# TritonDataCenter/containerpilot

Hardware: AMD Instinct MI355X
Metric: events/sec (higher is better)
Workload: dtype n/a (CPU daemon, no tensor math; see BASELINE.json north_star); 1 GPU; model=containerpilot daemon, BASELINE stress shape scaled to 550 jobs, jobs=550, watches=50, parallelism=1 independent daemons (1/rank)

## Files before the change

cpp/include/cpilot/discovery.hpp:

```cpp
#pragma once

#include <condition_variable>
#include <deque>
#include <functional>
#include <map>
#include <memory>
#include <set>
#include <mutex>
#include <string>
#include <thread>
#include <vector>

#include "cpilot/http.hpp"
#include "cpilot/json.hpp"
#include "cpilot/kv.hpp"
#include "cpilot/loop.hpp"
#include "cpilot/metrics.hpp"

namespace cpilot {

struct ServiceEntry {
  std::string id;
  std::string address;
  int port = 0;
  std::vector<std::string> tags;
  std::string node;
  std::string nodeAddress;
};

std::vector<ServiceEntry> parseHealthEntries(const std::string& body,
                                             bool* ok);

std::string kvRequestPath(const std::string& key, bool prefix,
                          const std::string& dc, bool blocking = false,
                          uint64_t index = 0, int waitSeconds = 0);

class ConsulBackend {
 public:
  static std::unique_ptr<ConsulBackend> create(const Json* raw,
                                               std::string* err);

  ~ConsulBackend();

  void start(Loop& loop);
  void stop();

  using DoneCb = std::function<void(bool ok, const std::string& err)>;
  using HealthCb =
      std::function<void(bool ok, std::vector<ServiceEntry> entries)>;
  using HealthBlockingCb = std::function<void(
      bool ok, std::vector<ServiceEntry> entries, uint64_t index)>;

  void serviceRegister(const std::string& id, const std::string& name,
                       const std::vector<std::string>& tags, int port,
                       const std::string& address, bool enableTagOverride,
                       int ttlSeconds, const std::string& status,
                       const std::string& deregisterAfter, DoneCb cb);
  void updateTTL(const std::string& checkID, const std::string& output,
                 const std::string& status, DoneCb cb);
  void serviceDeregister(const std::string& id, DoneCb cb);
  void healthService(const std::string& name, const std::string& tag,
                     const std::string& dc, HealthCb cb);

  void healthServiceBlocking(const std::string& name, const std::string& tag,
                             const std::string& dc, uint64_t lastIndex,
                             int waitSeconds, HealthBlockingCb cb);

  bool compareAndSwap(const std::string& service,
                      std::vector<ServiceEntry> entries);

  using KVCb = std::function<void(bool ok, std::vector<KVEntry> entries)>;
  using KVBlockingCb = std::function<void(
      bool ok, std::vector<KVEntry> entries, uint64_t index)>;
  void kvGet(const std::string& key, bool prefix, const std::string& dc,
             KVCb cb);
  void kvGetBlocking(const std::string& key, bool prefix,
                     const std::string& dc, uint64_t lastIndex,
                     int waitSeconds, KVBlockingCb cb);
  bool compareAndSwapKV(const std::string& watch,
                        std::vector<KVEntry> entries);

  const std::string& address() const { return address_; }
  const std::string& scheme() const { return scheme_; }

  std::shared_ptr<prom::Family> watchGauge() { return watchGauge_; }

 private:
  ConsulBackend() = default;
  void workerMain();
  bool enqueue(const std::string& key, std::function<void()> task);
  using BlockingFinish = std::function<std::function<void()>(
      const http::ClientResult& res, bool live, uint64_t index)>;
  bool startBlockingGet(const std::string& path, int waitSeconds,
                        size_t maxBody, BlockingFinish finish);

  std::string address_;
  std::string scheme_ = "http";
  std::string token_;
  http::TlsOptions tls_;

  Loop* loop_ = nullptr;
  std::vector<std::thread> workers_;
  std::deque<std::pair<std::string, std::function<void()>>> tasks_;
  std::set<std::string> queuedKeys_;
  uint64_t dropped_ = 0;
  std::mutex mu_;
  std::condition_variable cv_;
  bool stopping_ = false;

  std::map<std::string, std::vector<ServiceEntry>> watched_;
  std::map<std::string, std::vector<KVEntry>> watchedKV_;
  std::shared_ptr<prom::Family> watchGauge_;

  struct BlockingReg {
    std::mutex mu;
    std::set<std::shared_ptr<http::CancelToken>> tokens;
    bool stopping = false;
  };
  std::shared_ptr<BlockingReg> blockingReg_ =
      std::make_shared<BlockingReg>();
};

struct ServiceDefinition
    : public std::enable_shared_from_this<ServiceDefinition> {
  std::string id;
  std::string name;
  int port = 0;
  int ttl = 0;
  std::vector<std::string> tags;
  std::string initialStatus;
  std::string ipAddress;
  bool enableTagOverride = false;
  std::string deregisterCriticalServiceAfter;
  ConsulBackend* consul = nullptr;

  bool wasRegistered = false;
  bool registerInFlight = false;

  void sendHeartbeat();
  void registerWithInitialStatus();
  void deregister();
  void markForMaintenance();

 private:
  void registerService(const std::string& status);
};

}
```

cpp/include/cpilot/http.hpp:

```cpp
#pragma once

#include <sys/socket.h>

#include <functional>
#include <map>
#include <mutex>
#include <memory>
#include <string>

#include "cpilot/loop.hpp"

namespace cpilot {
namespace http {

struct Request {
  std::string method;
  std::string path;
  std::string query;
  std::map<std::string, std::string> headers;
  std::string body;
};

struct Response {
  int status = 200;
// ... 61 lines not shown
class CancelToken {
 public:
  void arm(int fd);
  void disarm();
  void cancel();
  bool cancelled();

 private:
  std::mutex mu_;
  int fd_ = -1;
  bool cancelled_ = false;
};

struct TlsOptions {
  bool enabled = false;
  std::string caFile;
  std::string caPath;
  std::string certFile;
  std::string keyFile;
  std::string serverName;
  bool insecureSkipVerify = false;
};

extern const char* const kBodyTooLarge;

ClientResult request(const std::string& target, const std::string& method,
                     const std::string& path, const std::string& body,
                     const std::string& contentType = "application/json",
                     const std::map<std::string, std::string>& headers = {},
                     int timeoutMs = 10000,
                     const TlsOptions* tls = nullptr,
                     CancelToken* cancel = nullptr, size_t maxBody = 0);

}
}
```

cpp/include/cpilot/loop.hpp:

```cpp
#pragma once

#include <sys/types.h>

#include <chrono>
#include <cstdint>
#include <deque>
#include <functional>
#include <map>
#include <memory>
#include <mutex>
#include <queue>
#include <vector>

namespace cpilot {

using Clock = std::chrono::steady_clock;
using TimePoint = Clock::time_point;
using Ns = std::chrono::nanoseconds;

std::function<void()> timedItem(const char* tag, std::function<void()> fn);
void dumpItemTags();

void resetThreadScheduling();

class Loop {
 public:
  using FdCallback = std::function<void(uint32_t epollEvents)>;
  using TimerCallback = std::function<void()>;
  using ChildCallback = std::function<void(int waitStatus)>;

  Loop();
  ~Loop();

  Loop(const Loop&) = delete;
  Loop& operator=(const Loop&) = delete;

  void watchFd(int fd, uint32_t events, FdCallback cb);
  void modifyFd(int fd, uint32_t events);
  void unwatchFd(int fd);

  uint64_t addTimeout(Ns delay, TimerCallback cb);
  uint64_t addInterval(Ns interval, TimerCallback cb, Ns initialDelay = Ns(-1));
  void cancelTimer(uint64_t id);

  void defer(std::function<void()> fn);

  void post(std::function<void()> fn);

  void watchChild(pid_t pid, ChildCallback cb);
  void reapChildren();
  void notifyChildExit(pid_t pid, int status);

  static void postIfLive(Loop* loop, uint64_t id, std::function<void()> fn);
  uint64_t id() const { return id_; }

  void run();
  void stop();

  bool stopped() const { return stopped_; }

 private:
  struct Timer {
    uint64_t id;
    TimePoint deadline;
    Ns interval;
    TimerCallback cb;
    bool canceled = false;
  };
  struct TimerCmp {
    bool operator()(const std::shared_ptr<Timer>& a,
                    const std::shared_ptr<Timer>& b) const {
      return a->deadline > b->deadline;
    }
  };

  void armTimerFd();
  void fireDueTimers();
  void drainDeferred();
  void drainPosted();

  uint64_t id_ = 0;
  int epfd_ = -1;
  int timerfd_ = -1;
  int wakeupFds_[2] = {-1, -1};
  bool stopped_ = false;

  std::map<int, FdCallback> fdCallbacks_;
  std::priority_queue<std::shared_ptr<Timer>,
                      std::vector<std::shared_ptr<Timer>>, TimerCmp>
      timers_;
  std::map<uint64_t, std::shared_ptr<Timer>> timersById_;
  uint64_t nextTimerId_ = 1;

  std::deque<std::function<void()>> deferred_;

  std::mutex postedMu_;
  std::deque<std::function<void()>> posted_;

  std::map<pid_t, ChildCallback> children_;
  std::map<pid_t, int> unclaimedExits_;
};

}
```

cpp/include/cpilot/spawner.hpp:

```cpp
#pragma once

#include <sys/types.h>

#include <cstdint>
#include <deque>
#include <functional>
#include <map>
#include <memory>
#include <mutex>
#include <string>
#include <thread>
#include <vector>

#include "cpilot/loop.hpp"

namespace cpilot {

class Spawner {
 public:
  using SpawnCb = std::function<void(pid_t pid, int err)>;

  static Spawner& global();

  void spawn(Loop& loop, const std::string& execPath,
             const std::vector<std::string>& args,
             std::shared_ptr<const std::vector<std::string>> baseEnv,
             const std::vector<std::string>& extraEnv, int stdioFd,
             SpawnCb cb);

  int helperCount() const { return (int)helpers_.size(); }

  size_t backlog();
  bool overloaded();

 private:
  Spawner();
  struct Helper {
    int sock = -1;
    pid_t pid = -1;
    bool dead = false;
    std::deque<std::pair<std::vector<char>, int>> overflow;
    std::mutex sendMu;
  };
  struct Pending {
    Loop* loop;
    uint64_t loopId;
    SpawnCb cb;
    size_t helperIdx;
  };

  bool launchHelper(Helper* h);
  void flushOverflow(size_t idx);
  void readerMain();
  void handleMessage(size_t idx, const char* buf, size_t len);
  void helperDied(size_t idx);
  bool sendRequest(Helper& h, const std::vector<char>& buf, int fd);
  void wakeReader();

  std::string helperPath_;
  std::vector<std::unique_ptr<Helper>> helpers_;
  size_t nextHelper_ = 0;

  std::mutex mu_;
  std::map<uint32_t, Pending> pending_;
  uint32_t nextReqId_ = 1;
  std::map<pid_t, std::pair<Loop*, uint64_t>> pidLoops_;

  int wakeFds_[2] = {-1, -1};
  std::thread reader_;
};

}
```

cpp/src/discovery.cpp:

```cpp
#include "cpilot/discovery.hpp"

#include <algorithm>
#include <cstdlib>
#include <thread>

#include "cpilot/decode.hpp"
#include "cpilot/http.hpp"
#include "cpilot/log.hpp"

namespace cpilot {

namespace {

void parseRawURI(const std::string& raw, std::string* address,
                 std::string* scheme) {
  *scheme = "http";
  *address = raw;
  if (raw.rfind("http://", 0) == 0) {
    *address = raw.substr(7);
  } else if (raw.rfind("https://", 0) == 0) {
    *address = raw.substr(8);
    *scheme = "https";
  }
}

std::string urlEncode(const std::string& s) {
  std::string out;
  for (unsigned char c : s) {
    if (isalnum(c) || c == '-' || c == '_' || c == '.' || c == '~' ||
        c == ':' || c == '@') {
      out += c;
    } else {
      char buf[4];
// ... 93 lines not shown
  if (const char* v = getenv("CONSUL_CACERT"))
    if (v[0]) backend->tls_.caFile = v;
  if (const char* v = getenv("CONSUL_CAPATH"))
    if (v[0]) backend->tls_.caPath = v;
  if (const char* v = getenv("CONSUL_CLIENT_CERT"))
    if (v[0]) backend->tls_.certFile = v;
  if (const char* v = getenv("CONSUL_CLIENT_KEY"))
    if (v[0]) backend->tls_.keyFile = v;
  if (const char* v = getenv("CONSUL_TLS_SERVER_NAME"))
    if (v[0]) backend->tls_.serverName = v;
  if (const char* v = getenv("CONSUL_HTTP_SSL_VERIFY")) {
    std::string s2(v);
    for (auto& ch : s2) ch = tolower(ch);
    if (s2 == "1" || s2 == "true") backend->tls_.insecureSkipVerify = false;
    else if (s2 == "0" || s2 == "false")
      backend->tls_.insecureSkipVerify = true;
  }
  backend->tls_.enabled = (backend->scheme_ == "https");
  backend->watchGauge_ = prom::Registry::global().registerFamily(
      "containerpilot_watch_instances",
      "gauge of instances found for each ContainerPilot watch, partitioned "
      "by service",
      prom::MetricType::Gauge, {"service"});
  return backend;
}

ConsulBackend::~ConsulBackend() { stop(); }

void ConsulBackend::start(Loop& loop) {
  loop_ = &loop;
  stopping_ = false;
  if (blockingReg_->stopping)
    blockingReg_ = std::make_shared<BlockingReg>();
  for (int i = 0; i < 4; i++)
    workers_.emplace_back([this] { workerMain(); });
}

void ConsulBackend::stop() {
  {
    std::lock_guard<std::mutex> l(mu_);
    if (stopping_ && workers_.empty()) return;
    stopping_ = true;
  }
  {
    std::lock_guard<std::mutex> l(blockingReg_->mu);
    blockingReg_->stopping = true;
    for (auto& t : blockingReg_->tokens) t->cancel();
  }
  cv_.notify_all();
  for (auto& t : workers_) t.join();
  workers_.clear();
}

void ConsulBackend::workerMain() {
  resetThreadScheduling();
  while (true) {
    std::function<void()> task;
    {
      std::unique_lock<std::mutex> l(mu_);
      cv_.wait(l, [this] { return stopping_ || !tasks_.empty(); });
      if (stopping_ && tasks_.empty()) return;
      auto& front = tasks_.front();
      if (!front.first.empty()) queuedKeys_.erase(front.first);
      task = std::move(front.second);
      tasks_.pop_front();
    }
    task();
  }
}

bool ConsulBackend::enqueue(const std::string& key,
                            std::function<void()> task) {
  {
    std::lock_guard<std::mutex> l(mu_);
    if (stopping_) return false;
    if (!key.empty() && !queuedKeys_.insert(key).second) return false;
    if (tasks_.size() >= 10000) {
      if (++dropped_ % 1000 == 1)
        LOG_WARN("consul task queue full, dropping requests (%llu dropped)",
                 (unsigned long long)dropped_);
      if (!key.empty()) queuedKeys_.erase(key);
      return false;
    }
    tasks_.emplace_back(key, std::move(task));
  }
  cv_.notify_one();
  return true;
}
// ... 15 lines not shown
  payload.emplace_back("ID", Json(id));
  payload.emplace_back("Name", Json(name));
  if (!tags.empty()) {
    JsonArray tagArr;
    for (auto& t : tags) tagArr.push_back(Json(t));
    payload.emplace_back("Tags", Json(std::move(tagArr)));
  }
  payload.emplace_back("Port", Json((int64_t)port));
  payload.emplace_back("Address", Json(address));
  if (enableTagOverride)
    payload.emplace_back("EnableTagOverride", Json(true));
  payload.emplace_back("Check", Json(std::move(check)));
  std::string body = Json(std::move(payload)).dump();

  std::string target = address_;
  std::string token = token_;
  http::TlsOptions tls = tls_;
  Loop* loop = loop_;
  bool accepted = enqueue("reg:" + id, [target, token, tls, body, cb, loop] {
    std::map<std::string, std::string> headers;
    if (!token.empty()) headers["X-Consul-Token"] = token;
    auto res = http::request(target, "PUT", "/v1/agent/service/register",
                             body, "application/json", headers, 10000, &tls);
    bool ok = res.ok && res.status == 200;
    std::string err = res.ok ? ("status " + std::to_string(res.status) + ": " +
                                res.body)
                             : res.error;
    loop->post(timedItem("consul", [cb, ok, err] { cb(ok, ok ? "" : err); }));
  });
  if (!accepted)
    loop_->post([cb] { cb(false, "request coalesced or queue full"); });
}

void ConsulBackend::updateTTL(const std::string& checkID,
                              const std::string& output,
                              const std::string& status, DoneCb cb) {
  std::string st = status;
  if (st == "pass") st = "passing";
  else if (st == "warn") st = "warning";
  else if (st == "fail") st = "critical";
  JsonObject payload;
  payload.emplace_back("Status", Json(st));
  payload.emplace_back("Output", Json(output));
  std::string body = Json(std::move(payload)).dump();
  std::string path = "/v1/agent/check/update/" + urlEncode(checkID);

  std::string target = address_;
  std::string token = token_;
  http::TlsOptions tls = tls_;
  Loop* loop = loop_;
  bool accepted =
      enqueue("ttl:" + checkID, [target, token, tls, path, body, cb, loop] {
    std::map<std::string, std::string> headers;
    if (!token.empty()) headers["X-Consul-Token"] = token;
    auto res = http::request(target, "PUT", path, body, "application/json",
                             headers, 10000, &tls);
    bool ok = res.ok && res.status == 200;
    std::string err =
        res.ok ? ("status " + std::to_string(res.status) + ": " + res.body)
               : res.error;
    loop->post(timedItem("consul", [cb, ok, err] { cb(ok, ok ? "" : err); }));
  });
  if (!accepted) {
    (void)cb;
  }
}

void ConsulBackend::serviceDeregister(const std::string& id, DoneCb cb) {
  std::string path = "/v1/agent/service/deregister/" + urlEncode(id);
  std::string target = address_;
  std::string token = token_;
  http::TlsOptions tls = tls_;
  Loop* loop = loop_;
  bool accepted = enqueue("", [target, token, tls, path, cb, loop] {
    std::map<std::string, std::string> headers;
    if (!token.empty()) headers["X-Consul-Token"] = token;
    auto res = http::request(target, "PUT", path, "", "application/json",
                             headers, 10000, &tls);
    bool ok = res.ok && res.status == 200;
    std::string err =
        res.ok ? ("status " + std::to_string(res.status)) : res.error;
    loop->post(timedItem("consul", [cb, ok, err] { cb(ok, ok ? "" : err); }));
  });
  if (!accepted) loop_->post([cb] { cb(false, "queue full"); });
}

std::vector<ServiceEntry> parseHealthEntries(const std::string& body,
                                             bool* ok) {
  std::vector<ServiceEntry> entries;
  try {
    Json doc = parseJson5(body);
    if (doc.isArray()) {
      for (auto& e : doc.array()) {
        const Json* svc = e.find("Service");
        if (!svc || !svc->isObject()) continue;
        ServiceEntry entry;
        if (const Json* v = svc->find("ID"))
          if (v->isString()) entry.id = v->str();
// ... 185 lines not shown
      });
  if (!started) loop_->post([cb] { cb(false, {}, 0); });
}

bool ConsulBackend::compareAndSwapKV(const std::string& watch,
                                     std::vector<KVEntry> entries) {
  std::vector<KVEntry>& cached = watchedKV_[watch];
  bool changed = kvEntriesDiffer(cached, entries);
  cached = std::move(entries);
  return changed;
}

bool ConsulBackend::compareAndSwap(const std::string& service,
                                   std::vector<ServiceEntry> entries) {
  std::vector<ServiceEntry> existing = watched_[service];
  watched_[service] = entries;
  if (existing.size() != entries.size()) return true;
  auto byID = [](const ServiceEntry& a, const ServiceEntry& b) {
    return a.id < b.id;
  };
  std::sort(existing.begin(), existing.end(), byID);
  std::sort(entries.begin(), entries.end(), byID);
  for (size_t i = 0; i < existing.size(); i++) {
    if (existing[i].address != entries[i].address ||
        existing[i].port != entries[i].port)
      return true;
  }
  return false;
}


void ServiceDefinition::sendHeartbeat() {
  registerService("passing");
  std::string checkID = "service:" + id;
  consul->updateTTL(checkID, "ok", "pass", [](bool ok, const std::string& err) {
    if (!ok) LOG_WARN("service update TTL failed: %s", err.c_str());
  });
}

void ServiceDefinition::registerWithInitialStatus() {
  if (wasRegistered) return;
  std::string status;
  if (initialStatus == "passing") status = "passing";
  else if (initialStatus == "warning") status = "warning";
  else if (initialStatus == "critical") status = "critical";
  LOG_INFO("Registering service %s with initial status set to %s",
           name.c_str(), initialStatus.c_str());
  registerService(status);
}

void ServiceDefinition::registerService(const std::string& status) {
  if (wasRegistered || registerInFlight) return;
  registerInFlight = true;
  std::weak_ptr<ServiceDefinition> weak = weak_from_this();
  consul->serviceRegister(
      id, name, tags, port, ipAddress, enableTagOverride, ttl, status,
      deregisterCriticalServiceAfter,
      [weak](bool ok, const std::string& err) {
        auto self = weak.lock();
        if (!self) return;
        self->registerInFlight = false;
        if (!ok) {
          LOG_WARN("service registration failed: %s", err.c_str());
          return;
        }
        LOG_INFO("Service registered: %s", self->name.c_str());
        self->wasRegistered = true;
      });
}

// ... 11 lines not shown
```

cpp/src/http.cpp:

```cpp
#include "cpilot/http.hpp"

#include <sys/epoll.h>

#include <arpa/inet.h>
#include <fcntl.h>
#include <netdb.h>
#include <netinet/in.h>
#include <netinet/tcp.h>
#include <poll.h>
#include <openssl/err.h>
#include <openssl/ssl.h>
#include <sys/socket.h>
#include <sys/un.h>
#include <unistd.h>

#include <cctype>
#include <cstring>

#include "cpilot/log.hpp"

namespace cpilot {
namespace http {

const char* statusText(int code) {
// ... 432 lines not shown
         SSL_CTX_use_PrivateKey_file(ctx, tls.keyFile.c_str(),
                                     SSL_FILETYPE_PEM) != 1)) {
      *err = "failed to load client certificate/key";
      return false;
    }
    SSL_CTX_set_verify(
        ctx, tls.insecureSkipVerify ? SSL_VERIFY_NONE : SSL_VERIFY_PEER,
        nullptr);
    ssl = SSL_new(ctx);
    SSL_set_fd(ssl, fd);
    std::string sniHost = tls.serverName.empty() ? host : tls.serverName;
    size_t colon = sniHost.rfind(':');
    if (colon != std::string::npos) sniHost = sniHost.substr(0, colon);
    SSL_set_tlsext_host_name(ssl, sniHost.c_str());
    if (!tls.insecureSkipVerify) SSL_set1_host(ssl, sniHost.c_str());
    if (SSL_connect(ssl) != 1) {
      unsigned long e = ERR_get_error();
      char ebuf[256];
      ERR_error_string_n(e, ebuf, sizeof(ebuf));
      *err = std::string("TLS handshake failed: ") + ebuf;
      return false;
    }
    return true;
  }

  ssize_t send(const char* data, size_t len) {
    return ssl ? SSL_write(ssl, data, (int)len) : write(fd, data, len);
  }
  ssize_t recv(char* data, size_t len) {
    return ssl ? SSL_read(ssl, data, (int)len) : read(fd, data, len);
  }
};

struct ConnPool {
  std::map<std::string, int> conns;
  ~ConnPool() {
    for (auto& kv : conns) close(kv.second);
  }
};
thread_local ConnPool connPool;

int poolTake(const std::string& target) {
  auto it = connPool.conns.find(target);
  if (it == connPool.conns.end()) return -1;
  int fd = it->second;
  connPool.conns.erase(it);
  return fd;
}

void poolStore(const std::string& target, int fd) {
  int& slot = connPool.conns.emplace(target, -1).first->second;
  if (slot >= 0) close(slot);
  slot = fd;
}

bool tryDechunk(const std::string& data, std::string* out) {
  out->clear();
  size_t pos = 0;
  while (true) {
    size_t eol = data.find("\r\n", pos);
    if (eol == std::string::npos) return false;
    long len = strtol(data.substr(pos, eol - pos).c_str(), nullptr, 16);
    if (len < 0) return false;
    if (len == 0) return true;
    if (data.size() < eol + 2 + (size_t)len + 2) return false;
    out->append(data, eol + 2, (size_t)len);
    pos = eol + 2 + (size_t)len + 2;
  }
}

int acquireConn(const std::string& target, int timeoutMs, bool usePool,
                bool* fromPool, std::string* err) {
  int fd = usePool ? poolTake(target) : -1;
  *fromPool = fd >= 0;
  if (fd < 0) fd = connectTarget(target, err);
  if (fd >= 0) setIoTimeout(fd, timeoutMs);
  return fd;
}

std::string serialiseRequest(const std::string& method, const std::string& path,
                             const std::string& host, bool keepAlive,
                             const Headers& headers, const std::string& body,
                             const std::string& contentType) {
  std::string req = method + " " + path + " HTTP/1.1\r\n";
  req += "Host: " + host + "\r\n";
  req += keepAlive ? "Connection: keep-alive\r\n" : "Connection: close\r\n";
  for (auto& kv : headers) req += kv.first + ": " + kv.second + "\r\n";
  if (!body.empty() || method == "POST" || method == "PUT") {
    req += "Content-Type: " + contentType + "\r\n";
    req += "Content-Length: " + std::to_string(body.size()) + "\r\n";
  }
  req += "\r\n";
  req += body;
  return req;
}

bool writeAll(Transport& t, const std::string& data) {
  size_t off = 0;
  while (off < data.size()) {
    ssize_t n = t.send(data.data() + off, data.size() - off);
    if (n > 0)
      off += n;
    else if (!(n < 0 && errno == EINTR && !t.ssl))
      return false;
  }
  return true;
}

bool readMore(Transport& t, std::string* resp) {
  char buf[8192];
// ... 28 lines not shown
  if (isChunked(result->headers)) {
    std::string decoded;
    while (!tryDechunk(resp.substr(bodyStart), &decoded)) {
      if (maxBody && decoded.size() > maxBody) return ReadResult::TooLarge;
      if (!readMore(t, &resp)) return ReadResult::Truncated;
    }
    if (maxBody && decoded.size() > maxBody) return ReadResult::TooLarge;
    result->body = std::move(decoded);
  } else if (result->headers.count("content-length")) {
    size_t want = contentLength(result->headers);
    if (maxBody && want > maxBody) return ReadResult::TooLarge;
    while (resp.size() < bodyStart + want) {
      if (!readMore(t, &resp)) return ReadResult::Truncated;
    }
    result->body = resp.substr(bodyStart, want);
  } else {
    while (readMore(t, &resp)) {
      if (maxBody && resp.size() - bodyStart > maxBody)
        return ReadResult::TooLarge;
    }
    result->body = resp.substr(bodyStart);
    *bodyFramed = false;
  }
  return ReadResult::Ok;
}

bool serverKeepsAlive(const ClientResult& result) {
  auto it = result.headers.find("connection");
  bool closes = it != result.headers.end() &&
                toLower(it->second).find("close") != std::string::npos;
  return !closes && result.status > 0;
}

}

ClientResult request(const std::string& target, const std::string& method,
                     const std::string& path, const std::string& body,
                     const std::string& contentType,
                     const std::map<std::string, std::string>& headers,
                     int timeoutMs, const TlsOptions* tls,
                     CancelToken* cancel, size_t maxBody) {
  ClientResult result;
  if (cancel && cancel->cancelled()) {
    result.error = "cancelled";
    return result;
  }
  const bool tlsOn = tls && tls->enabled;
  const bool reusable = !tlsOn && cancel == nullptr;
  const std::string host =
      target.rfind("unix:", 0) == 0 ? "localhost" : target;
  const std::string req = serialiseRequest(method, path, host, reusable,
                                           headers, body, contentType);

  for (int attempt = 0; attempt < 2; attempt++) {
    result = ClientResult{};
    Transport t;
    bool fromPool = false;
    t.fd = acquireConn(target, timeoutMs, reusable && attempt == 0, &fromPool,
                       &result.error);
    if (t.fd < 0) return result;
    struct Disarm {
      CancelToken* ct;
      ~Disarm() {
        if (ct) ct->disarm();
      }
    } disarm{cancel};
    if (cancel) cancel->arm(t.fd);
    if (tlsOn && !t.startTls(host, *tls, &result.error)) return result;

    if (!writeAll(t, req)) {
      if (fromPool) continue;
      break;
    }
    bool bodyFramed = false;
    ReadResult rr = readResponse(t, &result, &bodyFramed, maxBody);
    if (rr == ReadResult::Empty && fromPool)
      continue;
    if (rr == ReadResult::Empty || rr == ReadResult::Malformed) {
      result.error = (cancel && cancel->cancelled()) ? "cancelled"
                                                     : "malformed response";
      return result;
    }
    if (rr == ReadResult::Truncated) {
      result.error = "truncated response body";
      return result;
    }
    if (rr == ReadResult::TooLarge) {
      result.error = kBodyTooLarge;
      return result;
    }
    result.ok = true;
    if (reusable && bodyFramed && serverKeepsAlive(result)) {
      poolStore(target, t.fd);
      t.fd = -1;
    }
    return result;
  }
  result.error = "write failed";
  return result;
}

}
}
```

cpp/src/loop.cpp:

```cpp
#include "cpilot/loop.hpp"

#include <fcntl.h>
#include <sched.h>
#include <sys/resource.h>
#include <sys/epoll.h>
#include <sys/timerfd.h>
#include <sys/wait.h>
#include <unistd.h>

#include <cstdio>
#include <cstring>
#include <algorithm>
#include <set>
#include <stdexcept>

#include "cpilot/log.hpp"

namespace cpilot {

void resetThreadScheduling() {
  struct sched_param sp;
  memset(&sp, 0, sizeof(sp));
  sched_setscheduler(0, SCHED_OTHER, &sp);
  setpriority(PRIO_PROCESS, 0, 0);
}

namespace {
std::mutex& liveLoopsMu() {
  static std::mutex mu;
  return mu;
}
std::map<Loop*, uint64_t>& liveLoops() {
  static std::map<Loop*, uint64_t> loops;
  return loops;
}
uint64_t nextLoopId() {
  static uint64_t next = 1;
  return next++;
// ... 10 lines not shown
  return tags;
}
}

std::function<void()> timedItem(const char* tag, std::function<void()> fn) {
  static const bool on = cpilotDebugEnv("CPILOT_LOOP_DEBUG");
  if (!on) return fn;
  std::string t(tag);
  return [t, fn = std::move(fn)] {
    TimePoint t0 = Clock::now();
    fn();
    auto& slot = itemTags()[t];
    slot.ms +=
        std::chrono::duration<double, std::milli>(Clock::now() - t0).count();
    slot.count++;
  };
}

void dumpItemTags() {
  for (auto& kv : itemTags())
    fprintf(stderr, "  item tag %s: %.0fms over %llu (avg %.1fus)\n",
            kv.first.c_str(), kv.second.ms,
            (unsigned long long)kv.second.count,
            kv.second.count ? kv.second.ms * 1000 / kv.second.count : 0.0);
  itemTags().clear();
}

void Loop::postIfLive(Loop* loop, uint64_t id, std::function<void()> fn) {
  std::lock_guard<std::mutex> l(liveLoopsMu());
  auto it = liveLoops().find(loop);
  if (it != liveLoops().end() && it->second == id) loop->post(std::move(fn));
}

Loop::Loop() {
  {
    std::lock_guard<std::mutex> l(liveLoopsMu());
    id_ = nextLoopId();
    liveLoops()[this] = id_;
  }
  epfd_ = epoll_create1(EPOLL_CLOEXEC);
  if (epfd_ < 0) throw std::runtime_error("epoll_create1 failed");
  timerfd_ = timerfd_create(CLOCK_MONOTONIC, TFD_NONBLOCK | TFD_CLOEXEC);
  if (timerfd_ < 0) throw std::runtime_error("timerfd_create failed");
  if (pipe2(wakeupFds_, O_NONBLOCK | O_CLOEXEC) != 0)
    throw std::runtime_error("pipe2 failed");

  watchFd(timerfd_, EPOLLIN, [this](uint32_t) {
    uint64_t expirations;
    while (read(timerfd_, &expirations, sizeof(expirations)) > 0) {
    }
    fireDueTimers();
  });
  watchFd(wakeupFds_[0], EPOLLIN, [this](uint32_t) {
    char buf[256];
    while (read(wakeupFds_[0], buf, sizeof(buf)) > 0) {
    }
    drainPosted();
  });
}

Loop::~Loop() {
  {
    std::lock_guard<std::mutex> l(liveLoopsMu());
    liveLoops().erase(this);
  }
  if (epfd_ >= 0) close(epfd_);
  if (timerfd_ >= 0) close(timerfd_);
  if (wakeupFds_[0] >= 0) close(wakeupFds_[0]);
  if (wakeupFds_[1] >= 0) close(wakeupFds_[1]);
}

void Loop::watchFd(int fd, uint32_t events, FdCallback cb) {
  struct epoll_event ev;
  memset(&ev, 0, sizeof(ev));
  ev.events = events;
  ev.data.fd = fd;
  if (epoll_ctl(epfd_, EPOLL_CTL_ADD, fd, &ev) != 0)
    throw std::runtime_error(std::string("epoll_ctl ADD failed: ") +
                             strerror(errno));
  fdCallbacks_[fd] = std::move(cb);
}

void Loop::modifyFd(int fd, uint32_t events) {
  struct epoll_event ev;
  memset(&ev, 0, sizeof(ev));
  ev.events = events;
  ev.data.fd = fd;
  epoll_ctl(epfd_, EPOLL_CTL_MOD, fd, &ev);
}

void Loop::unwatchFd(int fd) {
  epoll_ctl(epfd_, EPOLL_CTL_DEL, fd, nullptr);
  fdCallbacks_.erase(fd);
}

uint64_t Loop::addTimeout(Ns delay, TimerCallback cb) {
  auto t = std::make_shared<Timer>();
  t->id = nextTimerId_++;
  t->deadline = Clock::now() + delay;
  t->interval = Ns(0);
  t->cb = std::move(cb);
  timersById_[t->id] = t;
  timers_.push(t);
  armTimerFd();
  return t->id;
}

uint64_t Loop::addInterval(Ns interval, TimerCallback cb, Ns initialDelay) {
  if (interval <= Ns(0)) interval = Ns(1);
  if (initialDelay < Ns(0)) initialDelay = interval;
  auto t = std::make_shared<Timer>();
  t->id = nextTimerId_++;
  t->deadline = Clock::now() + initialDelay;
  t->interval = interval;
  t->cb = std::move(cb);
  timersById_[t->id] = t;
  timers_.push(t);
  armTimerFd();
  return t->id;
}

void Loop::cancelTimer(uint64_t id) {
  auto it = timersById_.find(id);
  if (it == timersById_.end()) return;
  it->second->canceled = true;
  timersById_.erase(it);
}

void Loop::defer(std::function<void()> fn) { deferred_.push_back(std::move(fn)); }

void Loop::post(std::function<void()> fn) {
  {
    std::lock_guard<std::mutex> l(postedMu_);
    posted_.push_back(std::move(fn));
  }
  char b = 1;
  ssize_t unused = write(wakeupFds_[1], &b, 1);
  (void)unused;
}

void Loop::watchChild(pid_t pid, ChildCallback cb) {
  auto it = unclaimedExits_.find(pid);
  if (it != unclaimedExits_.end()) {
    int status = it->second;
    unclaimedExits_.erase(it);
    cb(status);
    return;
  }
  children_[pid] = std::move(cb);
}

void Loop::reapChildren() {
  constexpr int kReapBatch = 64;
  int n = 0;
  while (n < kReapBatch) {
    int status = 0;
    pid_t pid = waitpid(-1, &status, WNOHANG);
    if (pid <= 0) return;
    n++;
    notifyChildExit(pid, status);
  }
  defer([this] { reapChildren(); });
}

void Loop::notifyChildExit(pid_t pid, int status) {
  auto it = children_.find(pid);
  if (it != children_.end()) {
    ChildCallback cb = std::move(it->second);
    children_.erase(it);
    cb(status);
  } else {
// ... 82 lines not shown
      more = !posted_.empty();
    }
    static const bool itemDebug = cpilotDebugEnv("CPILOT_LOOP_DEBUG");
    if (itemDebug) {
      static double accMs = 0;
      static uint64_t nItems = 0, nSlow = 0;
      static TimePoint lastDump = Clock::now();
      for (auto& fn : batch) {
        TimePoint ti = Clock::now();
        fn();
        double ms = std::chrono::duration<double, std::milli>(
                        Clock::now() - ti).count();
        accMs += ms;
        nItems++;
        if (ms > 0.2) nSlow++;
      }
      if (Clock::now() - lastDump > std::chrono::seconds(5)) {
        fprintf(stderr,
                "posted items: %llu in 5s, total=%.0fms avg=%.1fus "
                "slow(>200us)=%llu\n",
                (unsigned long long)nItems, accMs,
                nItems ? accMs * 1000.0 / nItems : 0.0,
                (unsigned long long)nSlow);
        accMs = 0;
        nItems = nSlow = 0;
        lastDump = Clock::now();
      }
    } else {
      for (auto& fn : batch) fn();
    }
    processed += batch.size();
    if (batch.empty()) break;
  }
  if (more) {
    char b = 1;
    ssize_t unused = write(wakeupFds_[1], &b, 1);
    (void)unused;
  }
}

void Loop::run() {
  stopped_ = false;
  const bool stallDebug = cpilotDebugEnv("CPILOT_LOOP_DEBUG");
  auto probe = [stallDebug](const char* phase, TimePoint t0, int fd = -1) {
    if (!stallDebug) return;
    auto ms = std::chrono::duration<double, std::milli>(Clock::now() - t0)
                  .count();
    if (ms > 10.0)
      fprintf(stderr, "loop stall: %s fd=%d took %.1f ms\n", phase, fd, ms);
  };
  std::vector<struct epoll_event> events(64);
  double accDeferred = 0, accEpoll = 0, accFds = 0, accTimers = 0;
  std::map<int, std::pair<double, uint64_t>> accPerFd;
  uint64_t iters = 0;
  TimePoint lastReport = Clock::now();
  auto acc = [](double* slot, TimePoint t0) {
    *slot += std::chrono::duration<double, std::milli>(Clock::now() - t0)
                 .count();
  };
  while (!stopped_) {
    TimePoint t0 = Clock::now();
    drainDeferred();
    probe("drainDeferred", t0);
    if (stallDebug) acc(&accDeferred, t0);
    if (stopped_) break;
    armTimerFd();
    int timeoutMs = deferred_.empty() ? 1000 : 0;
    TimePoint te = Clock::now();
    int n = epoll_wait(epfd_, events.data(), (int)events.size(), timeoutMs);
    if (stallDebug) acc(&accEpoll, te);
    if (n < 0) {
// ... 58 lines not shown
```

cpp/src/spawner.cpp:

```cpp
#include "cpilot/spawner.hpp"

#include <fcntl.h>
#include <limits.h>
#include <poll.h>
#include <signal.h>
#include <spawn.h>
#include <string.h>
#include <sys/socket.h>
#include <unistd.h>

#include <cstdio>
#include <cstdlib>

#include "cpilot/log.hpp"
#include "cpilot/spawnproto.hpp"

extern char** environ;

namespace cpilot {

using namespace spawnproto;

namespace {

int defaultHelperCount() {
  if (const char* v = getenv("CPILOT_SPAWN_HELPERS")) {
    int n = atoi(v);
    if (n >= 1 && n <= 64) return n;
  }
  long ncpu = sysconf(_SC_NPROCESSORS_ONLN);
  if (ncpu < 1) ncpu = 1;
  int n = (int)(ncpu / 16);
  if (n < 2) n = 2;
  if (n > 8) n = 8;
  return n;
}

// ... 210 lines not shown
  if (stdioFd >= 0) close(stdioFd);
}

bool Spawner::sendRequest(Helper& h, const std::vector<char>& buf, int fd) {
  struct iovec iov{const_cast<char*>(buf.data()), buf.size()};
  struct msghdr msg;
  memset(&msg, 0, sizeof(msg));
  msg.msg_iov = &iov;
  msg.msg_iovlen = 1;
  char cmsgBuf[CMSG_SPACE(sizeof(int))];
  if (fd >= 0) {
    memset(cmsgBuf, 0, sizeof(cmsgBuf));
    msg.msg_control = cmsgBuf;
    msg.msg_controllen = sizeof(cmsgBuf);
    struct cmsghdr* c = CMSG_FIRSTHDR(&msg);
    c->cmsg_level = SOL_SOCKET;
    c->cmsg_type = SCM_RIGHTS;
    c->cmsg_len = CMSG_LEN(sizeof(int));
    memcpy(CMSG_DATA(c), &fd, sizeof(int));
  }
  while (true) {
    ssize_t n = sendmsg(h.sock, &msg, MSG_NOSIGNAL);
    if (spawnDebug())
      fprintf(stderr, "[spawner] sendmsg fd=%d n=%zd errno=%d\n", h.sock, n,
              n < 0 ? errno : 0);
    if (n >= 0) return true;
    if (errno == EINTR) continue;
    return false;
  }
}

void Spawner::readerMain() {
  resetThreadScheduling();
  std::vector<char> buf(64);
  while (true) {
    std::vector<struct pollfd> fds;
    {
      std::lock_guard<std::mutex> l(mu_);
      for (auto& h : helpers_) {
        short ev = h->dead ? 0 : POLLIN;
        if (!h->dead && !h->overflow.empty()) ev |= POLLOUT;
        fds.push_back({h->sock, ev, 0});
      }
    }
    fds.push_back({wakeFds_[0], POLLIN, 0});
    int rc = poll(fds.data(), (nfds_t)fds.size(), 1000);
    if (spawnDebug() && rc != 0) {
      fprintf(stderr, "[spawner] poll rc=%d", rc);
      for (size_t i = 0; i < fds.size(); i++)
        fprintf(stderr, " fd%d=%x", fds[i].fd, fds[i].revents);
      fprintf(stderr, "\n");
    }
    if (rc < 0) {
      if (errno == EINTR) continue;
      return;
    }
    if (fds.back().revents & POLLIN) {
      char drain[256];
      while (read(wakeFds_[0], drain, sizeof(drain)) > 0) {
      }
    }
    for (size_t i = 0; i + 1 < fds.size(); i++) {
      if (fds[i].revents & POLLOUT) flushOverflow(i);
      if (fds[i].revents & (POLLIN | POLLHUP | POLLERR)) {
        while (true) {
          ssize_t n = recv(fds[i].fd, buf.data(), buf.size(), MSG_DONTWAIT);
          if (n > 0) {
            if (spawnDebug())
              fprintf(stderr, "[spawner] msg from helper %zu len=%zd\n", i, n);
            handleMessage(i, buf.data(), (size_t)n);
            continue;
          }
          if (n < 0 && (errno == EAGAIN || errno == EINTR)) break;
          if (spawnDebug())
            fprintf(stderr, "[spawner] helper %zu died n=%zd errno=%d\n",
                    i, n, errno);
          helperDied(i);
          break;
        }
      }
    }
  }
}

void Spawner::handleMessage(size_t idx, const char* data, size_t len) {
  uint32_t type = 0;
  if (len >= sizeof(uint32_t)) memcpy(&type, data, sizeof(type));
  if (spawnDebug() && type != kSpawnReply && type != kChildExit)
    fprintf(stderr, "[spawner] DROP unknown msg type=%u len=%zu\n", type, len);
  if (type == kSpawnReply && len >= sizeof(Reply)) {
    Reply r;
    memcpy(&r, data, sizeof(r));
    Pending p;
    {
      std::lock_guard<std::mutex> l(mu_);
      auto it = pending_.find(r.reqId);
      if (it == pending_.end()) {
        if (spawnDebug())
          fprintf(stderr, "[spawner] DROP reply for unknown req %u\n",
                  r.reqId);
        return;
      }
      p = std::move(it->second);
      pending_.erase(it);
    }
    if (spawnDebug())
      fprintf(stderr, "[spawner] reply req %u pid %d\n", r.reqId, r.pid);
    if (r.pid > 0) pidLoops_[r.pid] = {p.loop, p.loopId};
    SpawnCb cb = std::move(p.cb);
    pid_t pid = r.pid;
    int err = r.err;
    Loop::postIfLive(p.loop, p.loopId,
                     timedItem("spawncb", [cb, pid, err] { cb(pid, err); }));
  } else if (type == kChildExit && len >= sizeof(ExitNotice)) {
    ExitNotice note;
    memcpy(&note, data, sizeof(note));
    auto it = pidLoops_.find(note.pid);
    if (it == pidLoops_.end()) {
      if (spawnDebug())
        fprintf(stderr, "[spawner] DROP exit notice for unknown pid %d\n",
                note.pid);
      return;
    }
    if (spawnDebug())
      fprintf(stderr, "[spawner] exit pid %d\n", note.pid);
    auto [loop, loopId] = it->second;
    pidLoops_.erase(it);
    pid_t pid = note.pid;
    int status = note.status;
    Loop::postIfLive(loop, loopId, timedItem("exit", [loop, pid, status] {
                       loop->notifyChildExit(pid, status);
                     }));
  }
}

void Spawner::helperDied(size_t idx) {
  std::vector<Pending> lost;
  {
    std::lock_guard<std::mutex> l(mu_);
    Helper& h = *helpers_[idx];
    if (h.dead) return;
    h.dead = true;
    LOG_ERROR("spawner: helper %d (pid %d) died; respawning",
              (int)idx, (int)h.pid);
    for (auto it = pending_.begin(); it != pending_.end();) {
      if (it->second.helperIdx == idx) {
        lost.push_back(std::move(it->second));
        it = pending_.erase(it);
      } else {
        ++it;
      }
    }
    for (auto& [obuf, ofd] : h.overflow)
      if (ofd >= 0) close(ofd);
    h.overflow.clear();
    close(h.sock);
    if (!launchHelper(&h)) {
      LOG_ERROR("spawner: helper respawn failed: %s", strerror(errno));
      h.dead = true;
    }
  }
  for (auto& p : lost) {
    SpawnCb cb = std::move(p.cb);
    Loop::postIfLive(p.loop, p.loopId, [cb] { cb(-1, ECHILD); });
  }
// ... 4 lines not shown
```

Baseline: 10990 events/s.

## Batch spawner posts, use eventfd wakeups, pre-serialise TTL heartbeats, cache socket timeouts

The spawner reader now collects callbacks per loop and posts them in batches. Loop wakeups move from a pipe to an eventfd and only fire when the posted queue goes from empty to non-empty. TTL heartbeat requests are serialised once per service and reused, pooled connections remember their IO timeout so setsockopt is skipped, and worker threads get names. Together these aim to cut syscalls, allocations and lock traffic per event. The cost is extra complexity, and callbacks may reach the loop slightly later when a batch is held back.

```diff
diff --git a/cpp/include/cpilot/discovery.hpp b/cpp/include/cpilot/discovery.hpp
--- a/cpp/include/cpilot/discovery.hpp
+++ b/cpp/include/cpilot/discovery.hpp
@@ -56,8 +56,16 @@
                        const std::string& address, bool enableTagOverride,
                        int ttlSeconds, const std::string& status,
                        const std::string& deregisterAfter, DoneCb cb);
-  void updateTTL(const std::string& checkID, const std::string& output,
-                 const std::string& status, DoneCb cb);
+  struct PreparedTTL {
+    std::string key;
+    std::string bytes;
+    std::function<void(const std::string& err)> onFailure;
+  };
+  std::shared_ptr<const PreparedTTL> prepareTTL(
+      const std::string& checkID, const std::string& output,
+      const std::string& status,
+      std::function<void(const std::string& err)> onFailure);
+  void updateTTL(const std::shared_ptr<const PreparedTTL>& prepared);
   void serviceDeregister(const std::string& id, DoneCb cb);
   void healthService(const std::string& name, const std::string& tag,
                      const std::string& dc, HealthCb cb);
@@ -87,7 +95,7 @@
 
  private:
   ConsulBackend() = default;
-  void workerMain();
+  void workerMain(int index);
   bool enqueue(const std::string& key, std::function<void()> task);
   using BlockingFinish = std::function<std::function<void()>(
       const http::ClientResult& res, bool live, uint64_t index)>;
@@ -98,6 +106,7 @@
   std::string scheme_ = "http";
   std::string token_;
   http::TlsOptions tls_;
+  std::shared_ptr<const http::Endpoint> endpoint_;
 
   Loop* loop_ = nullptr;
   std::vector<std::thread> workers_;
@@ -144,6 +153,7 @@
 
  private:
   void registerService(const std::string& status);
+  std::shared_ptr<const ConsulBackend::PreparedTTL> heartbeat_;
 };
 
 }
diff --git a/cpp/include/cpilot/http.hpp b/cpp/include/cpilot/http.hpp
--- a/cpp/include/cpilot/http.hpp
+++ b/cpp/include/cpilot/http.hpp
@@ -117,5 +117,19 @@
                      const TlsOptions* tls = nullptr,
                      CancelToken* cancel = nullptr, size_t maxBody = 0);
 
+
+struct Endpoint {
+  std::string target;
+  TlsOptions tls;
+};
+
+std::string prepareRequest(const Endpoint& endpoint, const std::string& method,
+                           const std::string& path, const std::string& body,
+                           const std::string& contentType = "application/json",
+                           const Headers& headers = {});
+
+ClientResult sendPrepared(const Endpoint& endpoint, const std::string& bytes,
+                          int timeoutMs = 10000, size_t maxBody = 0);
+
 }
 }
diff --git a/cpp/include/cpilot/loop.hpp b/cpp/include/cpilot/loop.hpp
--- a/cpp/include/cpilot/loop.hpp
+++ b/cpp/include/cpilot/loop.hpp
@@ -50,8 +50,11 @@
   void watchChild(pid_t pid, ChildCallback cb);
   void reapChildren();
   void notifyChildExit(pid_t pid, int status);
+  size_t unclaimedExitCount() const { return unclaimedExits_.size(); }
 
   static void postIfLive(Loop* loop, uint64_t id, std::function<void()> fn);
+  static void postBatchIfLive(Loop* loop, uint64_t id,
+                              std::vector<std::function<void()>> items);
   uint64_t id() const { return id_; }
 
   void run();
@@ -78,11 +81,12 @@
   void fireDueTimers();
   void drainDeferred();
   void drainPosted();
+  void wake();
 
   uint64_t id_ = 0;
   int epfd_ = -1;
   int timerfd_ = -1;
-  int wakeupFds_[2] = {-1, -1};
+  int wakeFd_ = -1;
   bool stopped_ = false;
 
   std::map<int, FdCallback> fdCallbacks_;
diff --git a/cpp/include/cpilot/spawner.hpp b/cpp/include/cpilot/spawner.hpp
--- a/cpp/include/cpilot/spawner.hpp
+++ b/cpp/include/cpilot/spawner.hpp
@@ -54,6 +54,8 @@
   void readerMain();
   void handleMessage(size_t idx, const char* buf, size_t len);
   void helperDied(size_t idx);
+  void queuePost(Loop* loop, uint64_t loopId, std::function<void()> fn);
+  void flushPosts();
   bool sendRequest(Helper& h, const std::vector<char>& buf, int fd);
   void wakeReader();
 
@@ -66,6 +68,13 @@
   uint32_t nextReqId_ = 1;
   std::map<pid_t, std::pair<Loop*, uint64_t>> pidLoops_;
 
+  struct PostBatch {
+    Loop* loop;
+    uint64_t loopId;
+    std::vector<std::function<void()>> items;
+  };
+  std::vector<PostBatch> batches_;
+
   int wakeFds_[2] = {-1, -1};
   std::thread reader_;
 };
diff --git a/cpp/src/discovery.cpp b/cpp/src/discovery.cpp
--- a/cpp/src/discovery.cpp
+++ b/cpp/src/discovery.cpp
@@ -1,4 +1,6 @@
 #include "cpilot/discovery.hpp"
+
+#include <pthread.h>
 
 #include <algorithm>
 #include <cstdlib>
@@ -158,8 +160,12 @@
   stopping_ = false;
   if (blockingReg_->stopping)
     blockingReg_ = std::make_shared<BlockingReg>();
+  auto endpoint = std::make_shared<http::Endpoint>();
+  endpoint->target = address_;
+  endpoint->tls = tls_;
+  endpoint_ = std::move(endpoint);
   for (int i = 0; i < 4; i++)
-    workers_.emplace_back([this] { workerMain(); });
+    workers_.emplace_back([this, i] { workerMain(i); });
 }
 
 void ConsulBackend::stop() {
@@ -178,8 +184,10 @@
   workers_.clear();
 }
 
-void ConsulBackend::workerMain() {
+void ConsulBackend::workerMain(int index) {
   resetThreadScheduling();
+  pthread_setname_np(pthread_self(),
+                     ("cp-consul-" + std::to_string(index)).c_str());
   while (true) {
     std::function<void()> task;
     {
@@ -261,9 +269,10 @@
     loop_->post([cb] { cb(false, "request coalesced or queue full"); });
 }
 
-void ConsulBackend::updateTTL(const std::string& checkID,
-                              const std::string& output,
-                              const std::string& status, DoneCb cb) {
+std::shared_ptr<const ConsulBackend::PreparedTTL> ConsulBackend::prepareTTL(
+    const std::string& checkID, const std::string& output,
+    const std::string& status,
+    std::function<void(const std::string& err)> onFailure) {
   std::string st = status;
   if (st == "pass") st = "passing";
   else if (st == "warn") st = "warning";
@@ -271,28 +280,30 @@
   JsonObject payload;
   payload.emplace_back("Status", Json(st));
   payload.emplace_back("Output", Json(output));
-  std::string body = Json(std::move(payload)).dump();
-  std::string path = "/v1/agent/check/update/" + urlEncode(checkID);
-
-  std::string target = address_;
-  std::string token = token_;
-  http::TlsOptions tls = tls_;
+  http::Headers headers;
+  if (!token_.empty()) headers["X-Consul-Token"] = token_;
+  auto prepared = std::make_shared<PreparedTTL>();
+  prepared->key = "ttl:" + checkID;
+  prepared->bytes = http::prepareRequest(
+      *endpoint_, "PUT", "/v1/agent/check/update/" + urlEncode(checkID),
+      Json(std::move(payload)).dump(), "application/json", headers);
+  prepared->onFailure = std::move(onFailure);
+  return prepared;
+}
+
+void ConsulBackend::updateTTL(
+    const std::shared_ptr<const PreparedTTL>& prepared) {
   Loop* loop = loop_;
-  bool accepted =
-      enqueue("ttl:" + checkID, [target, token, tls, path, body, cb, loop] {
-    std::map<std::string, std::string> headers;
-    if (!token.empty()) headers["X-Consul-Token"] = token;
-    auto res = http::request(target, "PUT", path, body, "application/json",
-                             headers, 10000, &tls);
-    bool ok = res.ok && res.status == 200;
+  enqueue(prepared->key, [endpoint = endpoint_, prepared, loop] {
+    auto res = http::sendPrepared(*endpoint, prepared->bytes, 10000);
+    if (res.ok && res.status == 200) return;
     std::string err =
         res.ok ? ("status " + std::to_string(res.status) + ": " + res.body)
                : res.error;
-    loop->post(timedItem("consul", [cb, ok, err] { cb(ok, ok ? "" : err); }));
+    loop->post(timedItem("consul", [prepared, err] {
+      if (prepared->onFailure) prepared->onFailure(err);
+    }));
   });
-  if (!accepted) {
-    (void)cb;
-  }
 }
 
 void ConsulBackend::serviceDeregister(const std::string& id, DoneCb cb) {
@@ -544,10 +555,12 @@
 
 void ServiceDefinition::sendHeartbeat() {
   registerService("passing");
-  std::string checkID = "service:" + id;
-  consul->updateTTL(checkID, "ok", "pass", [](bool ok, const std::string& err) {
-    if (!ok) LOG_WARN("service update TTL failed: %s", err.c_str());
-  });
+  if (!heartbeat_)
+    heartbeat_ = consul->prepareTTL(
+        "service:" + id, "ok", "pass", [](const std::string& err) {
+          LOG_WARN("service update TTL failed: %s", err.c_str());
+        });
+  consul->updateTTL(heartbeat_);
 }
 
 void ServiceDefinition::registerWithInitialStatus() {
diff --git a/cpp/src/http.cpp b/cpp/src/http.cpp
--- a/cpp/src/http.cpp
+++ b/cpp/src/http.cpp
@@ -488,26 +488,31 @@
   }
 };
 
+struct PooledConn {
+  int fd = -1;
+  int timeoutMs = -1;
+};
 struct ConnPool {
-  std::map<std::string, int> conns;
+  std::map<std::string, PooledConn> conns;
   ~ConnPool() {
-    for (auto& kv : conns) close(kv.second);
+    for (auto& kv : conns)
+      if (kv.second.fd >= 0) close(kv.second.fd);
   }
 };
 thread_local ConnPool connPool;
 
-int poolTake(const std::string& target) {
+PooledConn poolTake(const std::string& target) {
   auto it = connPool.conns.find(target);
-  if (it == connPool.conns.end()) return -1;
-  int fd = it->second;
-  connPool.conns.erase(it);
-  return fd;
-}
-
-void poolStore(const std::string& target, int fd) {
-  int& slot = connPool.conns.emplace(target, -1).first->second;
-  if (slot >= 0) close(slot);
-  slot = fd;
+  if (it == connPool.conns.end()) return PooledConn{};
+  PooledConn conn = it->second;
+  it->second = PooledConn{};
+  return conn;
+}
+
+void poolStore(const std::string& target, PooledConn conn) {
+  PooledConn& slot = connPool.conns[target];
+  if (slot.fd >= 0) close(slot.fd);
+  slot = conn;
 }
 
 bool tryDechunk(const std::string& data, std::string* out) {
@@ -527,11 +532,17 @@
 
 int acquireConn(const std::string& target, int timeoutMs, bool usePool,
                 bool* fromPool, std::string* err) {
-  int fd = usePool ? poolTake(target) : -1;
-  *fromPool = fd >= 0;
-  if (fd < 0) fd = connectTarget(target, err);
-  if (fd >= 0) setIoTimeout(fd, timeoutMs);
-  return fd;
+  PooledConn conn = usePool ? poolTake(target) : PooledConn{};
+  *fromPool = conn.fd >= 0;
+  if (conn.fd < 0) conn.fd = connectTarget(target, err);
+  if (conn.fd >= 0 && conn.timeoutMs != timeoutMs)
+    setIoTimeout(conn.fd, timeoutMs);
+  return conn.fd;
+}
+
+const std::string& hostHeader(const std::string& target) {
+  static const std::string localhost = "localhost";
+  return target.rfind("unix:", 0) == 0 ? localhost : target;
 }
 
 std::string serialiseRequest(const std::string& method, const std::string& path,
@@ -626,26 +637,12 @@
   return !closes && result.status > 0;
 }
 
-}
-
-ClientResult request(const std::string& target, const std::string& method,
-                     const std::string& path, const std::string& body,
-                     const std::string& contentType,
-                     const std::map<std::string, std::string>& headers,
-                     int timeoutMs, const TlsOptions* tls,
-                     CancelToken* cancel, size_t maxBody) {
+ClientResult exchange(const std::string& target, const std::string& host,
+                      const std::string& req, bool reusable, int timeoutMs,
+                      const TlsOptions* tls, CancelToken* cancel,
+                      size_t maxBody) {
   ClientResult result;
-  if (cancel && cancel->cancelled()) {
-    result.error = "cancelled";
-    return result;
-  }
   const bool tlsOn = tls && tls->enabled;
-  const bool reusable = !tlsOn && cancel == nullptr;
-  const std::string host =
-      target.rfind("unix:", 0) == 0 ? "localhost" : target;
-  const std::string req = serialiseRequest(method, path, host, reusable,
-                                           headers, body, contentType);
-
   for (int attempt = 0; attempt < 2; attempt++) {
     result = ClientResult{};
     Transport t;
@@ -685,7 +682,7 @@
     }
     result.ok = true;
     if (reusable && bodyFramed && serverKeepsAlive(result)) {
-      poolStore(target, t.fd);
+      poolStore(target, PooledConn{t.fd, timeoutMs});
       t.fd = -1;
     }
     return result;
@@ -695,4 +692,40 @@
 }
 
 }
-}
+
+ClientResult request(const std::string& target, const std::string& method,
+                     const std::string& path, const std::string& body,
+                     const std::string& contentType,
+                     const std::map<std::string, std::string>& headers,
+                     int timeoutMs, const TlsOptions* tls,
+                     CancelToken* cancel, size_t maxBody) {
+  if (cancel && cancel->cancelled()) {
+    ClientResult result;
+    result.error = "cancelled";
+    return result;
+  }
+  const bool reusable = !(tls && tls->enabled) && cancel == nullptr;
+  const std::string& host = hostHeader(target);
+  return exchange(target, host,
+                  serialiseRequest(method, path, host, reusable, headers, body,
+                                   contentType),
+                  reusable, timeoutMs, tls, cancel, maxBody);
+}
+
+std::string prepareRequest(const Endpoint& endpoint, const std::string& method,
+                           const std::string& path, const std::string& body,
+                           const std::string& contentType,
+                           const Headers& headers) {
+  return serialiseRequest(method, path, hostHeader(endpoint.target),
+                          !endpoint.tls.enabled, headers, body, contentType);
+}
+
+ClientResult sendPrepared(const Endpoint& endpoint, const std::string& bytes,
+                          int timeoutMs, size_t maxBody) {
+  return exchange(endpoint.target, hostHeader(endpoint.target), bytes,
+                  !endpoint.tls.enabled, timeoutMs, &endpoint.tls, nullptr,
+                  maxBody);
+}
+
+}
+}
diff --git a/cpp/src/loop.cpp b/cpp/src/loop.cpp
--- a/cpp/src/loop.cpp
+++ b/cpp/src/loop.cpp
@@ -4,6 +4,7 @@
 #include <sched.h>
 #include <sys/resource.h>
 #include <sys/epoll.h>
+#include <sys/eventfd.h>
 #include <sys/timerfd.h>
 #include <sys/wait.h>
 #include <unistd.h>
@@ -80,6 +81,21 @@
   if (it != liveLoops().end() && it->second == id) loop->post(std::move(fn));
 }
 
+void Loop::postBatchIfLive(Loop* loop, uint64_t id,
+                           std::vector<std::function<void()>> items) {
+  if (items.empty()) return;
+  std::lock_guard<std::mutex> l(liveLoopsMu());
+  auto it = liveLoops().find(loop);
+  if (it == liveLoops().end() || it->second != id) return;
+  bool wasEmpty;
+  {
+    std::lock_guard<std::mutex> pl(loop->postedMu_);
+    wasEmpty = loop->posted_.empty();
+    for (auto& fn : items) loop->posted_.push_back(std::move(fn));
+  }
+  if (wasEmpty) loop->wake();
+}
+
 Loop::Loop() {
   {
     std::lock_guard<std::mutex> l(liveLoopsMu());
@@ -90,8 +106,8 @@
   if (epfd_ < 0) throw std::runtime_error("epoll_create1 failed");
   timerfd_ = timerfd_create(CLOCK_MONOTONIC, TFD_NONBLOCK | TFD_CLOEXEC);
   if (timerfd_ < 0) throw std::runtime_error("timerfd_create failed");
-  if (pipe2(wakeupFds_, O_NONBLOCK | O_CLOEXEC) != 0)
-    throw std::runtime_error("pipe2 failed");
+  wakeFd_ = eventfd(0, EFD_NONBLOCK | EFD_CLOEXEC);
+  if (wakeFd_ < 0) throw std::runtime_error("eventfd failed");
 
   watchFd(timerfd_, EPOLLIN, [this](uint32_t) {
     uint64_t expirations;
@@ -99,10 +115,10 @@
     }
     fireDueTimers();
   });
-  watchFd(wakeupFds_[0], EPOLLIN, [this](uint32_t) {
-    char buf[256];
-    while (read(wakeupFds_[0], buf, sizeof(buf)) > 0) {
-    }
+  watchFd(wakeFd_, EPOLLIN, [this](uint32_t) {
+    uint64_t count;
+    ssize_t unused = read(wakeFd_, &count, sizeof(count));
+    (void)unused;
     drainPosted();
   });
 }
@@ -114,8 +130,7 @@
   }
   if (epfd_ >= 0) close(epfd_);
   if (timerfd_ >= 0) close(timerfd_);
-  if (wakeupFds_[0] >= 0) close(wakeupFds_[0]);
-  if (wakeupFds_[1] >= 0) close(wakeupFds_[1]);
+  if (wakeFd_ >= 0) close(wakeFd_);
 }
 
 void Loop::watchFd(int fd, uint32_t events, FdCallback cb) {
@@ -177,14 +192,20 @@
 
 void Loop::defer(std::function<void()> fn) { deferred_.push_back(std::move(fn)); }
 
+void Loop::wake() {
+  uint64_t one = 1;
+  ssize_t unused = write(wakeFd_, &one, sizeof(one));
+  (void)unused;
+}
+
 void Loop::post(std::function<void()> fn) {
+  bool wasEmpty;
   {
     std::lock_guard<std::mutex> l(postedMu_);
+    wasEmpty = posted_.empty();
     posted_.push_back(std::move(fn));
   }
-  char b = 1;
-  ssize_t unused = write(wakeupFds_[1], &b, 1);
-  (void)unused;
+  if (wasEmpty) wake();
 }
 
 void Loop::watchChild(pid_t pid, ChildCallback cb) {
@@ -333,11 +354,7 @@
     processed += batch.size();
     if (batch.empty()) break;
   }
-  if (more) {
-    char b = 1;
-    ssize_t unused = write(wakeupFds_[1], &b, 1);
-    (void)unused;
-  }
+  if (more) wake();
 }
 
 void Loop::run() {
diff --git a/cpp/src/spawner.cpp b/cpp/src/spawner.cpp
--- a/cpp/src/spawner.cpp
+++ b/cpp/src/spawner.cpp
@@ -3,6 +3,7 @@
 #include <fcntl.h>
 #include <limits.h>
 #include <poll.h>
+#include <pthread.h>
 #include <signal.h>
 #include <spawn.h>
 #include <string.h>
@@ -279,6 +280,7 @@
 
 void Spawner::readerMain() {
   resetThreadScheduling();
+  pthread_setname_np(pthread_self(), "cp-spawn-rd");
   std::vector<char> buf(64);
   while (true) {
     std::vector<struct pollfd> fds;
@@ -322,12 +324,34 @@
           if (spawnDebug())
             fprintf(stderr, "[spawner] helper %zu died n=%zd errno=%d\n",
                     i, n, errno);
+          flushPosts();
           helperDied(i);
           break;
         }
       }
     }
-  }
+    flushPosts();
+  }
+}
+
+void Spawner::queuePost(Loop* loop, uint64_t loopId,
+                        std::function<void()> fn) {
+  constexpr size_t kMaxBatch = 256;
+  for (auto& b : batches_) {
+    if (b.loop == loop && b.loopId == loopId) {
+      b.items.push_back(std::move(fn));
+      if (b.items.size() >= kMaxBatch) flushPosts();
+      return;
+    }
+  }
+  batches_.push_back(PostBatch{loop, loopId, {}});
+  batches_.back().items.push_back(std::move(fn));
+}
+
+void Spawner::flushPosts() {
+  for (auto& b : batches_)
+    Loop::postBatchIfLive(b.loop, b.loopId, std::move(b.items));
+  batches_.clear();
 }
 
 void Spawner::handleMessage(size_t idx, const char* data, size_t len) {
@@ -357,8 +381,8 @@
     SpawnCb cb = std::move(p.cb);
     pid_t pid = r.pid;
     int err = r.err;
-    Loop::postIfLive(p.loop, p.loopId,
-                     timedItem("spawncb", [cb, pid, err] { cb(pid, err); }));
+    queuePost(p.loop, p.loopId,
+              timedItem("spawncb", [cb, pid, err] { cb(pid, err); }));
   } else if (type == kChildExit && len >= sizeof(ExitNotice)) {
     ExitNotice note;
     memcpy(&note, data, sizeof(note));
@@ -375,9 +399,9 @@
     pidLoops_.erase(it);
     pid_t pid = note.pid;
     int status = note.status;
-    Loop::postIfLive(loop, loopId, timedItem("exit", [loop, pid, status] {
-                       loop->notifyChildExit(pid, status);
-                     }));
+    queuePost(loop, loopId, timedItem("exit", [loop, pid, status] {
+                loop->notifyChildExit(pid, status);
+              }));
   }
 }
 
```

New measurement: 11000 events/s, median of 2. No clear change (+0.0%).
